# stcodeer/Frequency-wised_All-in-One_Image_Restoration_Model

Measured on AMD Instinct MI355X. Metric: training images/sec @128x128, higher is better.
Workload: dtype bf16; 1 GPU; BASELINE configs[1]: Uformer encoder+decoder (all_3_bands, L=3, freq MSA), denoise sigma=25, 128x128, phase-2 train step (fwd+bwd+Adam, DropPath on); per_gpu_batch=16, global_batch=16, parallelism=dp1, hip_graph=True

## Files before the change

### frequency-wised_all-in-one_image_restoration_model_amd/csrc/fw_common.h

```cpp
#pragma once
#include <hip/hip_runtime.h>
#include <stdint.h>
#include <mutex>

#define FW_DT_F32 0
#define FW_DT_BF16 1

typedef __attribute__((ext_vector_type(4))) float f32x4;
typedef __attribute__((ext_vector_type(8))) __bf16 bf16x8_t;
typedef unsigned short bf16raw;

#define FW_DEV static __device__ __forceinline__
#define FW_SPEC __device__ __forceinline__
#define FW_MEM __device__ __forceinline__

FW_DEV int lane_id() { return threadIdx.x & 63; }

FW_DEV float bf2f(bf16raw b) { return __uint_as_float(((unsigned)b) << 16); }
FW_DEV bf16raw f2bf(float f) {
    __bf16 h = (__bf16)f;
    return __builtin_bit_cast(bf16raw, h);
}
typedef __attribute__((ext_vector_type(2))) float fw_f32x2;
typedef __attribute__((ext_vector_type(2))) __bf16 fw_bf16x2;
FW_DEV unsigned pack_bf2(float lo, float hi) {
    const fw_f32x2 v = {lo, hi};
    return __builtin_bit_cast(unsigned, __builtin_convertvector(v, fw_bf16x2));
}

template <typename T> struct TT;
template <> struct TT<float> {
    static constexpr int SZ = 4;
    static constexpr int E16 = 4;
    FW_DEV float ld(const float* p) { return *p; }
    FW_DEV void st(float* p, float v) { *p = v; }
};
template <> struct TT<bf16raw> {
    static constexpr int SZ = 2;
    static constexpr int E16 = 8;
    FW_DEV float ld(const bf16raw* p) { return bf2f(*p); }
    FW_DEV void st(bf16raw* p, float v) { *p = f2bf(v); }
};

template <typename T> FW_DEV void unpack16(const uint4& v, float* f);
template <> FW_SPEC void unpack16<float>(const uint4& v, float* f) {
    f[0] = __uint_as_float(v.x); f[1] = __uint_as_float(v.y);
    f[2] = __uint_as_float(v.z); f[3] = __uint_as_float(v.w);
}
template <> FW_SPEC void unpack16<bf16raw>(const uint4& v, float* f) {
    f[0] = __uint_as_float(v.x << 16); f[1] = __uint_as_float(v.x & 0xffff0000u);
    f[2] = __uint_as_float(v.y << 16); f[3] = __uint_as_float(v.y & 0xffff0000u);
    f[4] = __uint_as_float(v.z << 16); f[5] = __uint_as_float(v.z & 0xffff0000u);
    f[6] = __uint_as_float(v.w << 16); f[7] = __uint_as_float(v.w & 0xffff0000u);
}
template <typename T> FW_DEV uint4 pack16(const float* f);
template <> FW_SPEC uint4 pack16<float>(const float* f) {
    return make_uint4(__float_as_uint(f[0]), __float_as_uint(f[1]), __float_as_uint(f[2]), __float_as_uint(f[3]));
}
template <> FW_SPEC uint4 pack16<bf16raw>(const float* f) {
    return make_uint4(pack_bf2(f[0], f[1]), pack_bf2(f[2], f[3]), pack_bf2(f[4], f[5]), pack_bf2(f[6], f[7]));
}

FW_DEV float erf_fast(float x) {
    const float ax = fabsf(x);
    const float t = __builtin_amdgcn_rcpf(1.0f + 0.3275911f * ax);
    const float poly = t * (0.254829592f + t * (-0.284496736f + t * (1.421413741f + t * (-1.453152027f + t * 1.061405429f))));
    const float r = 1.0f - poly * __expf(-ax * ax);
    return copysignf(r, x);
}
FW_DEV float gelu_f(float x) { return 0.5f * x * (1.0f + erf_fast(x * 0.70710678118654752440f)); }
FW_DEV float gelu_grad_f(float x) {
    const float cdf = 0.5f * (1.0f + erf_fast(x * 0.70710678118654752440f));
    const float pdf = 0.39894228040143267794f * __expf(-0.5f * x * x);
    return cdf + x * pdf;
}
FW_DEV float gelu_poly(float x) {
    const float xc = __builtin_amdgcn_fmed3f(x, -4.0f, 4.0f);
    const float u = xc * xc;
    float p = -1.301290697e-09f;
    p = fmaf(p, u, 1.041962340e-07f); p = fmaf(p, u, -3.657149647e-06f); p = fmaf(p, u, 7.485542814e-05f);
    p = fmaf(p, u, -1.006494109e-03f); p = fmaf(p, u, 9.505412949e-03f); p = fmaf(p, u, -6.588785358e-02f);
    p = fmaf(p, u, 3.986733717e-01f);
    return x * fmaf(xc, p, 0.5f);
}
FW_DEV float gelu_grad_poly(float x) {
    const float xc = __builtin_amdgcn_fmed3f(x, -4.0f, 4.0f);
    const float u = xc * xc;
    float r = -1.641741003e-08f;
    r = fmaf(r, u, 1.213663647e-06f); r = fmaf(r, u, -3.845618281e-05f); r = fmaf(r, u, 6.876052189e-04f);
    r = fmaf(r, u, -7.687198903e-03f); r = fmaf(r, u, 5.591419208e-02f); r = fmaf(r, u, -2.620297180e-01f);
    r = fmaf(r, u, 7.967230048e-01f);
    return fmaf(xc, r, 0.5f);
}
template <typename T> FW_DEV float gelu_t(float x) { return sizeof(T) == 2 ? gelu_poly(x) : gelu_f(x); }
template <typename T> FW_DEV float gelu_grad_t(float x) { return sizeof(T) == 2 ? gelu_grad_poly(x) : gelu_grad_f(x); }
FW_DEV float lrelu_f(float x, float s) { return x > 0.f ? x : x * s; }

FW_DEV float wave_sum(float v) {
#pragma unroll
    for (int o = 32; o > 0; o >>= 1) v += __shfl_xor(v, o, 64);
    return v;
}
FW_DEV float wave_max(float v) {
#pragma unroll
    for (int o = 32; o > 0; o >>= 1) v = fmaxf(v, __shfl_xor(v, o, 64));
    return v;
}

FW_DEV unsigned fw_hash32(unsigned x) {
    x ^= x >> 16; x *= 0x7feb352dU; x ^= x >> 15; x *= 0x846ca68bU; x ^= x >> 16;
    return x;
}
FW_DEV unsigned fw_site_key(unsigned seed, unsigned site) { return fw_hash32(seed ^ fw_hash32(site * 0x9E3779B9U + 0x7F4A7C15U)); }
FW_DEV bool fw_keep(unsigned key, unsigned long long idx, unsigned thresh) {
    return fw_hash32(fw_hash32((unsigned)idx ^ key) + (unsigned)(idx >> 32)) >= thresh;
}
static inline unsigned fw_drop_thresh(float p) {
    const double t = (double)p * 4294967296.0;
    return t <= 0.0 ? 0u : (t >= 4294967295.0 ? 4294967295u : (unsigned)t);
}

template <typename T> FW_DEV void mma_chunk(f32x4& acc, const uint4& a, const uint4& b);
template <> FW_SPEC void mma_chunk<bf16raw>(f32x4& acc, const uint4& a, const uint4& b) {
    acc = __builtin_amdgcn_mfma_f32_16x16x32_bf16(__builtin_bit_cast(bf16x8_t, a),
                                                  __builtin_bit_cast(bf16x8_t, b), acc, 0, 0, 0);
}
template <> FW_SPEC void mma_chunk<float>(f32x4& acc, const uint4& a, const uint4& b) {
    acc = __builtin_amdgcn_mfma_f32_16x16x4f32(__uint_as_float(a.x), __uint_as_float(b.x), acc, 0, 0, 0);
    acc = __builtin_amdgcn_mfma_f32_16x16x4f32(__uint_as_float(a.y), __uint_as_float(b.y), acc, 0, 0, 0);
    acc = __builtin_amdgcn_mfma_f32_16x16x4f32(__uint_as_float(a.z), __uint_as_float(b.z), acc, 0, 0, 0);
    acc = __builtin_amdgcn_mfma_f32_16x16x4f32(__uint_as_float(a.w), __uint_as_float(b.w), acc, 0, 0, 0);
}

FW_DEV uint4 frag_kc(const char* tile, int ldb, int row0, int chunk) {
    const int l = lane_id();
    return *reinterpret_cast<const uint4*>(tile + (row0 + (l & 15)) * ldb + chunk * 64 + ((l >> 4) << 4));
}

template <typename T> FW_DEV uint4 frag_km(const char* tile, int ldb, int m0, int chunk);
template <> FW_SPEC uint4 frag_km<float>(const char* tile, int ldb, int m0, int chunk) {
    const int l = lane_id();
    const char* p = tile + (chunk * 16 + ((l >> 4) << 2)) * ldb + (m0 + (l & 15)) * 4;
    uint4 r;
    r.x = *reinterpret_cast<const unsigned*>(p);
    r.y = *reinterpret_cast<const unsigned*>(p + ldb);
    r.z = *reinterpret_cast<const unsigned*>(p + 2 * ldb);
    r.w = *reinterpret_cast<const unsigned*>(p + 3 * ldb);
    return r;
}
typedef __attribute__((ext_vector_type(4))) short fw_s16x4;
typedef __attribute__((address_space(3))) fw_s16x4 fw_lds_s16x4;
template <> FW_SPEC uint4 frag_km<bf16raw>(const char* tile, int ldb, int m0, int chunk) {
    const int l = lane_id();
    const char* p = tile + (chunk * 32 + ((l >> 4) << 3) + ((l >> 2) & 3)) * ldb + (m0 + ((l & 3) << 2)) * 2;
    const uint2 lo = __builtin_bit_cast(uint2, __builtin_amdgcn_ds_read_tr16_b64_v4i16((fw_lds_s16x4*)p));
    const uint2 hi = __builtin_bit_cast(uint2, __builtin_amdgcn_ds_read_tr16_b64_v4i16((fw_lds_s16x4*)(p + 4 * ldb)));
    return make_uint4(lo.x, lo.y, hi.x, hi.y);
}

template <typename T> FW_DEV void store_acc_T(char* dst, int ldb, int row0, int col0, const f32x4& acc);
template <> FW_SPEC void store_acc_T<float>(char* dst, int ldb, int row0, int col0, const f32x4& acc) {
    const int l = lane_id();
    *reinterpret_cast<f32x4*>(dst + (col0 + (l & 15)) * ldb + (row0 + ((l >> 4) << 2)) * 4) = acc;
}
template <> FW_SPEC void store_acc_T<bf16raw>(char* dst, int ldb, int row0, int col0, const f32x4& acc) {
    const int l = lane_id();
    uint2 v = make_uint2(pack_bf2(acc[0], acc[1]), pack_bf2(acc[2], acc[3]));
    *reinterpret_cast<uint2*>(dst + (col0 + (l & 15)) * ldb + (row0 + ((l >> 4) << 2)) * 2) = v;
}
template <typename T> FW_DEV void store_acc_N(char* dst, int ldb, int row0, int col0, const f32x4& acc) {
    const int l = lane_id();
    char* p = dst + (row0 + ((l >> 4) << 2)) * ldb + (col0 + (l & 15)) * TT<T>::SZ;
#pragma unroll
    for (int r = 0; r < 4; ++r) TT<T>::st(reinterpret_cast<T*>(p + r * ldb), acc[r]);
}

template <typename T, int MT, int NT>
FW_DEV void mma_tiles(f32x4 (&acc)[MT][NT], const char* A, int lda, int a_row0, const char* B, int ldb,
// ... 41 lines not shown
```

### frequency-wised_all-in-one_image_restoration_model_amd/csrc/fw_elem.hip

```cpp
#include "fw_common.h"
#include <stdlib.h>

namespace {

constexpr int TPB = 256;
FW_DEV long gtid() { return (long)blockIdx.x * TPB + threadIdx.x; }
FW_DEV long gstride() { return (long)gridDim.x * TPB; }
static inline int grid_for(long n, int cap = 8192) { long g = (n + TPB - 1) / TPB; return (int)(g < 1 ? 1 : (g > cap ? cap : g)); }

template <typename T> FW_DEV void ldvec(const T* p, float* f) {
    unpack16<T>(*reinterpret_cast<const uint4*>(p), f);
}
template <typename T> FW_DEV void stvec(T* p, const float* f) { *reinterpret_cast<uint4*>(p) = pack16<T>(f); }
template <typename T> FW_DEV void ldvec4(const T* p, float* f);
template <> FW_SPEC void ldvec4<float>(const float* p, float* f) { unpack16<float>(*reinterpret_cast<const uint4*>(p), f); }
template <> FW_SPEC void ldvec4<bf16raw>(const bf16raw* p, float* f) {
    const uint2 v = *reinterpret_cast<const uint2*>(p);
    f[0] = __uint_as_float(v.x << 16); f[1] = __uint_as_float(v.x & 0xffff0000u);
    f[2] = __uint_as_float(v.y << 16); f[3] = __uint_as_float(v.y & 0xffff0000u);
}
template <typename T> FW_DEV void stvec4(T* p, const float* f);
template <> FW_SPEC void stvec4<float>(float* p, const float* f) { *reinterpret_cast<uint4*>(p) = pack16<float>(f); }
template <> FW_SPEC void stvec4<bf16raw>(bf16raw* p, const float* f) {
    *reinterpret_cast<uint2*>(p) = make_uint2(pack_bf2(f[0], f[1]), pack_bf2(f[2], f[3]));
}

template <typename T>
__global__ void cast_rows_kernel(const float* __restrict__ src, long lds_, T* __restrict__ dst, long ldd, long rows, int cols,
                                 const float* __restrict__ rowscale, int rps) {
    const int c4n = cols >> 2;
    for (long i = gtid(); i < rows * c4n; i += gstride()) {
        const long r = i / c4n; const int c = (int)(i % c4n) * 4;
        const f32x4 v = *reinterpret_cast<const f32x4*>(src + r * lds_ + c);
        const float s = rowscale ? rowscale[r / rps] : 1.f;
        T* d = dst + r * ldd + c;
        if (sizeof(T) == 4) *reinterpret_cast<f32x4*>(d) = v * s;
        else *reinterpret_cast<uint2*>(d) = make_uint2(pack_bf2(v[0] * s, v[1] * s), pack_bf2(v[2] * s, v[3] * s));
    }
}
__global__ void copy_rows_kernel(const float* __restrict__ src, long lds_, float* __restrict__ dst, long ldd, long rows, int cols, int acc) {
    const int c4n = cols >> 2;
    for (long i = gtid(); i < rows * c4n; i += gstride()) {
        const long r = i / c4n; const int c = (int)(i % c4n) * 4;
        f32x4 v = *reinterpret_cast<const f32x4*>(src + r * lds_ + c);
        if (acc) v += *reinterpret_cast<const f32x4*>(dst + r * ldd + c);
        *reinterpret_cast<f32x4*>(dst + r * ldd + c) = v;
    }
}
template <typename T>
__global__ void add_rows_kernel(const T* __restrict__ src, long lds_, T* __restrict__ dst, long ldd, long rows, int cols) {
    const int c4n = cols >> 2;
    for (long i = gtid(); i < rows * c4n; i += gstride()) {
        const long r = i / c4n; const int c = (int)(i % c4n) * 4;
        for (int e = 0; e < 4; ++e) {
            T* d = dst + r * ldd + c + e;
            TT<T>::st(d, TT<T>::ld(d) + TT<T>::ld(src + r * lds_ + c + e));
        }
    }
}
template <typename T>
__global__ void cast_flat_kernel(const float* __restrict__ src, T* __restrict__ dst, long n) {
    for (long i = gtid(); i < n; i += gstride()) TT<T>::st(dst + i, src[i]);
}
template <typename TI, typename TO>
__global__ void permute3_kernel(const TI* __restrict__ in, TO* __restrict__ out, int d0, int d1, int d2, long s0, long s1, long s2, int acc) {
    const long n = (long)d0 * d1 * d2;
    for (long i = gtid(); i < n; i += gstride()) {
        const int c = (int)(i % d2); const long t = i / d2; const int b = (int)(t % d1); const int a = (int)(t / d1);
        const long o = a * s0 + b * s1 + c * s2;
        float v = TT<TI>::ld(in + i);
        if (acc) v += TT<TO>::ld(out + o);
        TT<TO>::st(out + o, v);
    }
}

__global__ __launch_bounds__(256) void permute3_multi_kernel(const long long* __restrict__ tab, const long long* __restrict__ prefix, int num) {
    int lo = 0, hi = num;
    while (hi - lo > 1) {
        const int mid = (lo + hi) >> 1;
        if (prefix[mid] <= (long long)blockIdx.x) lo = mid; else hi = mid;
    }
    const long long* t = tab + (long)lo * 10;
    const float* src = reinterpret_cast<const float*>(t[0]);
    const int d1 = (int)t[3], d2 = (int)t[4];
// ... 240 lines not shown
    float gw[10][E];
#pragma unroll
    for (int k = 0; k < 10; ++k)
#pragma unroll
        for (int e = 0; e < E; ++e) gw[k][e] = 0.f;
    if (live)
        for (long s = s0; s < nstrips && s < s0 + NSTRIP; ++s) {
            const int sx = (int)(s % ns); const int y = (int)((s / ns) % H); const long b = s / ((long)ns * H);
            const int x0 = sx * SX;
            const bool left_ok = x0 > 0, right_ok = x0 + SX < W;
            const int xl = left_ok ? x0 - 1 : 0, xr = right_ok ? x0 + SX : W - 1;
            Raw4<T> rg[SX], raw[3][SX + 2];
            const T* grow = g1 + ((b * H + y) * W + x0) * ld1 + c0;
#pragma unroll
            for (int o = 0; o < SX; ++o) rg[o].load(grow + (long)o * ld1);
#pragma unroll
            for (int ky = 0; ky < 3; ++ky) {
                int yy = y - ky + 1;
                yy = yy < 0 ? 0 : (yy >= H ? H - 1 : yy);
                const T* row = dh2 + ((b * H + yy) * W) * ldg + c0;
                raw[ky][0].load(row + (long)xl * ldg);
#pragma unroll
                for (int cx = 0; cx < SX; ++cx) raw[ky][cx + 1].load(row + (long)(x0 + cx) * ldg);
                raw[ky][SX + 1].load(row + (long)xr * ldg);
            }
            float g[SX][E];
#pragma unroll
            for (int o = 0; o < SX; ++o) {
                rg[o].unpack(g[o]);
                if constexpr (GIN) {
#pragma unroll
                    for (int e = 0; e < E; ++e) g[o][e] = gelu_t<T>(g[o][e]);
                }
            }
#pragma unroll
            for (int ky = 0; ky < 3; ++ky) {
                const bool row_ok = (y - ky + 1 >= 0) && (y - ky + 1 < H);
#pragma unroll
                for (int j = 0; j < SX + 2; ++j) {
                    Raw4<T> r = raw[ky][j];
                    r.zero_unless(row_ok && (j >= 1 || left_ok) && (j <= SX || right_ok));
                    float d[E];
                    r.unpack(d);
                    if (ky == 1 && j >= 1 && j <= SX) {
#pragma unroll
                        for (int e = 0; e < E; ++e) gw[9][e] += d[e];
                    }
#pragma unroll
                    for (int kx = 0; kx < 3; ++kx) {
                        const int i = j + kx - 2;
                        if (i >= 0 && i < SX) {
#pragma unroll
                            for (int e = 0; e < E; ++e) gw[ky * 3 + kx][e] += g[i][e] * d[e];
                        }
                    }
                }
            }
        }
    __syncthreads();
#pragma unroll
    for (int k = 0; k < 10; ++k)
#pragma unroll
        for (int e = 0; e < E; ++e) {
            float sum = gw[k][e];
            sum += __shfl_xor(sum, 32, 64);
            if ((threadIdx.x & 63) < WG_VL) atomicAdd(&red[(vl * E + e) * 10 + k], sum);
        }
    __syncthreads();
    for (int i = threadIdx.x; i < WG_VL * E * 10; i += 256) {
        const int k = i % 10, ce = i / 10;
        const int c = (blockIdx.x % nvg) * WG_VL * E + ce;
        if (c < C) {
            if (k < 9) atomicAdd(dw + (long)c * 9 + k, red[i]);
            else atomicAdd(dbias + c, red[i]);
        }
    }
}

template <typename T, bool GIN>
__global__ __launch_bounds__(256, 3) void dwconv_fwd_pipe_kernel(const T* __restrict__ in, long ldi, const float* __restrict__ w, const float* __restrict__ bias,
                                                              T* __restrict__ out, T* __restrict__ out2, long ldo, int B, int H, int W, int C, int NT) {
    constexpr int SZ = TT<T>::SZ, E16 = TT<T>::E16;
    constexpr int PXB = DT_CB * SZ, ROWB = (DT_TX + 2) * PXB + 128, CHUNKS = PXB / 16;
    constexpr int NPIECE = (DT_TY + 2) * (DT_TX + 2) * CHUNKS, NI = (NPIECE + 255) / 256;
    constexpr int TILEB = (DT_TY + 2) * ROWB;
    extern __shared__ __attribute__((aligned(16))) char dsm[];
    const int ncb = (C + DT_CB - 1) / DT_CB, ntx = (W + DT_TX - 1) / DT_TX, nty = H / DT_TY;
    const int ncol = ncb * ntx;
    const long nrow = (long)B * nty, nchunk = (nrow + NT - 1) / NT;
    long bid = blockIdx.x;
    if ((gridDim.x & 7) == 0) bid = (long)(blockIdx.x & 7) * (gridDim.x >> 3) + (blockIdx.x >> 3);
    const int col = (int)(bid % ncol);
    const long chunk = bid / ncol;
    if (chunk >= nchunk) return;
    const int cb = col % ncb, tx = col / ncb;
    const long s0 = chunk * NT, s1 = s0 + NT < nrow ? s0 + NT : nrow;
    const int x0 = tx * DT_TX, c0b = cb * DT_CB;
    int ppack[NI], pxo[NI];
    unsigned pokm = 0;
#pragma unroll
    for (int i = 0; i < NI; ++i) {
        const int idx = threadIdx.x + i * 256;
        const int ch = idx % CHUNKS, px = (idx / CHUNKS) % (DT_TX + 2), row = (idx / (CHUNKS * (DT_TX + 2))) % (DT_TY + 2);
        int xx = x0 + px - 1, cc = c0b + ch * E16;
        if (idx < NPIECE && xx >= 0 && xx < W && cc + E16 <= C) pokm |= 1u << i;
        xx = xx < 0 ? 0 : (xx >= W ? W - 1 : xx); cc = cc + E16 <= C ? cc : 0;
        pxo[i] = xx * (int)ldi + cc; ppack[i] = (row * ROWB + px * PXB + ch * 16) | (row << 24);
    }
    const int cv = threadIdx.x & 15, ry = (threadIdx.x >> 4) & 7, sxl = threadIdx.x >> 7;
    const int c0 = c0b + cv * 4;
    const bool c_ok = c0 + 4 <= C;
    const int cw = c_ok ? c0 : 0;
    const int ox0 = x0 + sxl * 8;
    float* wl = reinterpret_cast<float*>(dsm + TILEB);
    for (int i = threadIdx.x; i < 9 * DT_CB; i += 256) {
        const int c = c0b + (i % DT_CB);
        wl[i] = c < C ? w[(i / DT_CB) * C + c] : 0.f;
    }
    const f32x4 b4 = *reinterpret_cast<const f32x4*>(bias + cw);
    const int rowelems = W * (int)ldi;
    uint4 r[NI];
    auto issue = [&](long s) {
        const T* base = in + (s / nty) * H * (long)rowelems;
        const int y0 = (int)(s % nty) * DT_TY;
#pragma unroll
        for (int i = 0; i < NI; ++i) {
            int yy = y0 + (ppack[i] >> 24) - 1;
            yy = yy < 0 ? 0 : (yy >= H ? H - 1 : yy);
            r[i] = *reinterpret_cast<const uint4*>(base + (yy * rowelems + pxo[i]));
        }
    };
    issue(s0);
    for (long s = s0; s < s1; ++s) {
        const long b = s / nty;
        const int y0 = (int)(s % nty) * DT_TY;
#pragma unroll
        for (int i = 0; i < NI; ++i) {
            if (threadIdx.x + i * 256 >= NPIECE) continue;
            const int yy = y0 + (ppack[i] >> 24) - 1;
            uint4 piece = r[i];
            if constexpr (GIN) {
                float f[E16];
                unpack16<T>(piece, f);
#pragma unroll
                for (int e = 0; e < E16; ++e) f[e] = gelu_t<T>(f[e]);
                piece = pack16<T>(f);
            }
            *reinterpret_cast<uint4*>(dsm + (ppack[i] & 0xffffff)) = (((pokm >> i) & 1) && yy >= 0 && yy < H) ? piece : make_uint4(0, 0, 0, 0);
            __builtin_amdgcn_sched_barrier(0);
        }
        __syncthreads();
        if (s + 1 < s1) issue(s + 1);
        float acc[8][4];
#pragma unroll
        for (int o = 0; o < 8; ++o)
#pragma unroll
            for (int e = 0; e < 4; ++e) acc[o][e] = b4[e];
#pragma unroll 1
        for (int ky = 0; ky < 3; ++ky) {
            const char* rowp = dsm + (ry + ky) * ROWB + (sxl * 8) * PXB + cv * 4 * SZ;
            f32x4 wk[3];
#pragma unroll
            for (int kx = 0; kx < 3; ++kx) wk[kx] = *reinterpret_cast<const f32x4*>(wl + (ky * 3 + kx) * DT_CB + cv * 4);
#pragma unroll
            for (int cx = 0; cx < 10; ++cx) {
                Raw4<T> q;
                q.lds(rowp + cx * PXB);
                float f[4];
                q.unpack(f);
#pragma unroll
                for (int kx = 0; kx < 3; ++kx) {
                    const int o = cx - kx;
                    if (o >= 0 && o < 8) {
#pragma unroll
                        for (int e = 0; e < 4; ++e) acc[o][e] += f[e] * wk[kx][e];
                    }
                }
            }
        }
        const long tok0 = ((b * H + y0 + ry) * W + ox0) * ldo + c0;
#pragma unroll
        for (int o = 0; o < 8; ++o) {
            const bool ok = c_ok && ox0 + o < W;
            if (ok) stvec4<T>(out + tok0 + (long)o * ldo, acc[o]);
#pragma unroll
            for (int e = 0; e < 4; ++e) acc[o][e] = gelu_t<T>(acc[o][e]);
            if (ok) stvec4<T>(out2 + tok0 + (long)o * ldo, acc[o]);
        }
        __syncthreads();
    }
}

template <typename T>
__global__ __launch_bounds__(256, 2) void dwconv_bwd_fused_kernel(const T* __restrict__ dh2, long ldg, const T* __restrict__ h1, const float* __restrict__ w,
                                                               T* __restrict__ dh1, long ldo, float* __restrict__ dw, float* __restrict__ dbias,
                                                               int B, int H, int W, int C, int NT) {
    constexpr int SZ = TT<T>::SZ, E16 = TT<T>::E16;
    constexpr int PXB = DT_CB * SZ, ROWB = (DT_TX + 2) * PXB + 128, CHUNKS = PXB / 16;
    constexpr int NPIECE = (DT_TY + 2) * (DT_TX + 2) * CHUNKS, NI = (NPIECE + 255) / 256;
    extern __shared__ __attribute__((aligned(16))) char dsm[];
    const int ncb = (C + DT_CB - 1) / DT_CB, ntx = (W + DT_TX - 1) / DT_TX, nty = H / DT_TY;
    const int ncol = ncb * ntx;
    const long nrow = (long)B * nty, nchunk = (nrow + NT - 1) / NT;
    long bid = blockIdx.x;
    if ((gridDim.x & 7) == 0) bid = (long)(blockIdx.x & 7) * (gridDim.x >> 3) + (blockIdx.x >> 3);
    const int col = (int)(bid % ncol);
    const long chunk = bid / ncol;
    if (chunk >= nchunk) return;
    const int cb = col % ncb, tx = col / ncb;
    const long s0 = chunk * NT, s1 = s0 + NT < nrow ? s0 + NT : nrow;
    const int x0 = tx * DT_TX, c0b = cb * DT_CB;
    int ppack[NI], pxo[NI];
    unsigned pokm = 0;
#pragma unroll
    for (int i = 0; i < NI; ++i) {
        const int idx = threadIdx.x + i * 256;
        const int ch = idx % CHUNKS, px = (idx / CHUNKS) % (DT_TX + 2), row = (idx / (CHUNKS * (DT_TX + 2))) % (DT_TY + 2);
        int xx = x0 + px - 1, cc = c0b + ch * E16;
        if (idx < NPIECE && xx >= 0 && xx < W && cc + E16 <= C) pokm |= 1u << i;
        xx = xx < 0 ? 0 : (xx >= W ? W - 1 : xx); cc = cc + E16 <= C ? cc : 0;
        pxo[i] = xx * (int)ldg + cc; ppack[i] = (row * ROWB + px * PXB + ch * 16) | (row << 24);
    }
    const int cv = threadIdx.x & 15, ry = (threadIdx.x >> 4) & 7, sxl = threadIdx.x >> 7;
    const int c0 = c0b + cv * 4;
    const bool c_ok = c0 + 4 <= C;
    const int cw = c_ok ? c0 : 0;
    const int ox0 = x0 + sxl * 8;
    constexpr int TILEB = (DT_TY + 2) * ROWB;
    float* wl = reinterpret_cast<float*>(dsm + TILEB);
    float* part = wl + 9 * DT_CB;
    for (int i = threadIdx.x; i < 9 * DT_CB; i += 256) {
        const int k = i / DT_CB, c = c0b + (i % DT_CB);
        wl[i] = c < C ? w[(8 - k) * C + c] : 0.f;
    }
#pragma unroll
    for (int j = 0; j < 40; ++j) part[j * 256 + threadIdx.x] = 0.f;
    float gb[4] = {0.f, 0.f, 0.f, 0.f};
    uint4 r[NI];
    Raw4<T> pre[8];
    const int rowelems = W * (int)ldg;
    auto issue_halo = [&](long s) {
        const T* base = dh2 + (s / nty) * H * (long)rowelems;
        const int y0 = (int)(s % nty) * DT_TY;
#pragma unroll
        for (int i = 0; i < NI; ++i) {
            int yy = y0 + (ppack[i] >> 24) - 1;
            yy = yy < 0 ? 0 : (yy >= H ? H - 1 : yy);
            r[i] = *reinterpret_cast<const uint4*>(base + (yy * rowelems + pxo[i]));
        }
    };
    auto issue_pre = [&](long s) {
        const T* base = h1 + (s / nty) * H * (long)rowelems;
        const int yoff = ((int)(s % nty) * DT_TY + ry) * rowelems + cw;
#pragma unroll
        for (int o = 0; o < 8; ++o) {
            const int xx = ox0 + o < W ? ox0 + o : W - 1;
            pre[o].load(base + (yoff + xx * (int)ldg));
        }
    };
    issue_halo(s0);
    issue_pre(s0);
    for (long s = s0; s < s1; ++s) {
        const long b = s / nty;
        const int y0 = (int)(s % nty) * DT_TY;
#pragma unroll
        for (int i = 0; i < NI; ++i) {
            if (threadIdx.x + i * 256 >= NPIECE) continue;
            const int yy = y0 + (ppack[i] >> 24) - 1;
            *reinterpret_cast<uint4*>(dsm + (ppack[i] & 0xffffff)) = (((pokm >> i) & 1) && yy >= 0 && yy < H) ? r[i] : make_uint4(0, 0, 0, 0);
        }
        __syncthreads();
        float g[8][4], acc[8][4];
#pragma unroll
        for (int o = 0; o < 8; ++o) {
            float hc[4];
            pre[o].unpack(hc);
            const bool in = ox0 + o < W;
#pragma unroll
            for (int e = 0; e < 4; ++e) { g[o][e] = in ? gelu_t<T>(hc[e]) : 0.f; acc[o][e] = 0.f; }
            if (o & 1) __builtin_amdgcn_sched_barrier(0);
        }
#pragma unroll 1
        for (int ky = 0; ky < 3; ++ky) {
            const char* rowp = dsm + (ry + ky) * ROWB + (sxl * 8) * PXB + cv * 4 * SZ;
            f32x4 wk[3];
            float gk[3][4];
#pragma unroll
            for (int kx = 0; kx < 3; ++kx) {
                wk[kx] = *reinterpret_cast<const f32x4*>(wl + (ky * 3 + kx) * DT_CB + cv * 4);
#pragma unroll
                for (int e = 0; e < 4; ++e) gk[kx][e] = 0.f;
            }
            const float bsel = ky == 1 ? 1.f : 0.f;
#pragma unroll
            for (int cx = 0; cx < 10; ++cx) {
                Raw4<T> q;
                q.lds(rowp + cx * PXB);
                float f[4];
                q.unpack(f);
                if (cx >= 1 && cx <= 8) {
#pragma unroll
                    for (int e = 0; e < 4; ++e) gb[e] += bsel * f[e];
                }
#pragma unroll
                for (int kx = 0; kx < 3; ++kx) {
                    const int o = cx - kx;
                    if (o >= 0 && o < 8) {
#pragma unroll
                        for (int e = 0; e < 4; ++e) {
                            acc[o][e] += f[e] * wk[kx][e];
                            gk[kx][e] += f[e] * g[o][e];
                        }
                    }
                }
                if (cx == 4) __builtin_amdgcn_sched_barrier(0);
            }
#pragma unroll
            for (int kx = 0; kx < 3; ++kx)
#pragma unroll
                for (int e = 0; e < 4; ++e) part[((ky * 3 + kx) * 4 + e) * 256 + threadIdx.x] += gk[kx][e];
        }
        __builtin_amdgcn_sched_barrier(0);
        if (s + 1 < s1) issue_halo(s + 1);
        __builtin_amdgcn_sched_barrier(0);
        T* orow = dh1 + ((b * H + y0 + ry) * W + ox0) * ldo + c0;
#pragma unroll
        for (int o = 0; o < 8; ++o) {
            float hc[4];
            Raw4<T> again = pre[o];
            again.launder();
            again.unpack(hc);
#pragma unroll
            for (int e = 0; e < 4; ++e) acc[o][e] *= gelu_grad_t<T>(hc[e]);
            if (c_ok && ox0 + o < W) stvec4<T>(orow + (long)o * ldo, acc[o]);
            if (o & 1) __builtin_amdgcn_sched_barrier(0);
        }
        if (s + 1 < s1) issue_pre(s + 1);
        __syncthreads();
    }
    float* red = reinterpret_cast<float*>(dsm);
    const int wave = threadIdx.x >> 6;
#pragma unroll
    for (int j = 0; j < 40; ++j) {
        float v = j < 36 ? part[j * 256 + threadIdx.x] : gb[j - 36];
        v += __shfl_xor(v, 16, 64);
        v += __shfl_xor(v, 32, 64);
        if ((threadIdx.x & 63) < 16) red[(wave * 16 + cv) * 40 + j] = v;
    }
    __syncthreads();
    for (int i = threadIdx.x; i < 16 * 40; i += 256) {
        const int cvv = i / 40, j = i % 40, k = j >> 2, e = j & 3;
        const float sum = red[cvv * 40 + j] + red[(16 + cvv) * 40 + j] + red[(32 + cvv) * 40 + j] + red[(48 + cvv) * 40 + j];
        const int c = c0b + cvv * 4 + e;
        if (c < C) {
            if (k < 9) atomicAdd(dw + (long)c * 9 + (8 - k), sum);
            else atomicAdd(dbias + c, sum);
        }
    }
}

template <typename T>
__global__ void im2col4_kernel(const float* __restrict__ x, long ldx, T* __restrict__ col, int B, int H, int W, int C) {
    const int Ho = H / 2, Wo = W / 2, c4n = C >> 2;
    const long total = (long)B * Ho * Wo * 16 * c4n;
    for (long i = gtid(); i < total; i += gstride()) {
        const int c = (int)(i % c4n) * 4; long t = i / c4n;
        const int tap = (int)(t % 16); t /= 16;
        const int ox = (int)(t % Wo); const int oy = (int)((t / Wo) % Ho); const long b = t / ((long)Wo * Ho);
        const int iy = 2 * oy - 1 + (tap >> 2), ix = 2 * ox - 1 + (tap & 3);
        f32x4 v = f32x4{0.f, 0.f, 0.f, 0.f};
        if (iy >= 0 && iy < H && ix >= 0 && ix < W) v = *reinterpret_cast<const f32x4*>(x + ((b * H + iy) * W + ix) * ldx + c);
        T* d = col + (t * 16 + tap) * (long)C + c;
        if (sizeof(T) == 4) *reinterpret_cast<f32x4*>(d) = v;
        else *reinterpret_cast<uint2*>(d) = make_uint2(pack_bf2(v[0], v[1]), pack_bf2(v[2], v[3]));
    }
}
template <typename T>
__global__ void col2im4_kernel(const T* __restrict__ dcol, float* __restrict__ dx, long lddx, const float* __restrict__ dres, long ldr,
                               int B, int H, int W, int C) {
    const int Ho = H / 2, Wo = W / 2, c4n = C >> 2;
    const long total = (long)B * H * W * c4n;
    for (long i = gtid(); i < total; i += gstride()) {
        const int c = (int)(i % c4n) * 4; const long tok = i / c4n;
        const int x = (int)(tok % W); const int y = (int)((tok / W) % H); const long b = tok / ((long)W * H);
        f32x4 acc = f32x4{0.f, 0.f, 0.f, 0.f};
        if (dres) acc = *reinterpret_cast<const f32x4*>(dres + tok * ldr + c);
        for (int ky = (y + 1) & 1; ky < 4; ky += 2) {
            const int oy = (y + 1 - ky) / 2;
            if (y + 1 - ky < 0 || oy >= Ho) continue;
            for (int kx = (x + 1) & 1; kx < 4; kx += 2) {
                const int ox = (x + 1 - kx) / 2;
                if (x + 1 - kx < 0 || ox >= Wo) continue;
                const T* s = dcol + (((b * Ho + oy) * Wo + ox) * 16 + ky * 4 + kx) * (long)C + c;
                for (int e = 0; e < 4; ++e) acc[e] += TT<T>::ld(s + e);
            }
        }
        *reinterpret_cast<f32x4*>(dx + tok * lddx + c) = acc;
    }
}

template <typename T>
__global__ void pixel_shuffle_kernel(const T* __restrict__ g, const float* __restrict__ bias, float* __restrict__ out, long ldo,
                                     int B, int H, int W, int Cout) {
    const int c4n = Cout >> 2;
    const long total = (long)B * H * W * 4 * c4n;
    for (long i = gtid(); i < total; i += gstride()) {
        const int c = (int)(i % c4n) * 4; long t = i / c4n;
        const int q = (int)(t % 4); t /= 4;
        const int x = (int)(t % W); const int y = (int)((t / W) % H); const long b = t / ((long)W * H);
        const T* s = g + t * 4L * Cout + q * Cout + c;
        float* d = out + ((b * 2 * H + 2 * y + (q >> 1)) * 2 * W + 2 * x + (q & 1)) * ldo + c;
        f32x4 v;
        for (int e = 0; e < 4; ++e) v[e] = TT<T>::ld(s + e) + bias[c + e];
        *reinterpret_cast<f32x4*>(d) = v;
    }
}
template <typename T>
// ... 744 lines not shown
```

Baseline: 329.2 images/sec.

## Reuse halo rows via LDS ring buffer and packed fp32x2 math in dwconv kernels

The depthwise conv forward and backward pipeline kernels now keep the tile rows in an LDS ring buffer. When walking down the image they load only the DT_TY new rows and reuse the two overlap rows from the previous tile, loading a full top halo only at the first tile or at an image start. The stencil FMAs, the GELU polynomials and the GELU-gradient polynomials are rewritten on 2-wide float vectors so the compiler can emit packed fp32 instructions. The bias-grad row accumulation is specialised per ky so the bsel multiply is dropped for bf16. This cuts redundant global loads and ALU instruction count, but adds ring-index arithmetic and more complex control flow.

```diff
diff --git a/frequency-wised_all-in-one_image_restoration_model_amd/csrc/fw_common.h b/frequency-wised_all-in-one_image_restoration_model_amd/csrc/fw_common.h
--- a/frequency-wised_all-in-one_image_restoration_model_amd/csrc/fw_common.h
+++ b/frequency-wised_all-in-one_image_restoration_model_amd/csrc/fw_common.h
@@ -94,6 +94,53 @@
 }
 template <typename T> FW_DEV float gelu_t(float x) { return sizeof(T) == 2 ? gelu_poly(x) : gelu_f(x); }
 template <typename T> FW_DEV float gelu_grad_t(float x) { return sizeof(T) == 2 ? gelu_grad_poly(x) : gelu_grad_f(x); }
+FW_DEV fw_f32x2 fw_fma2(fw_f32x2 a, fw_f32x2 b, fw_f32x2 c) { return __builtin_elementwise_fma(a, b, c); }
+FW_DEV fw_f32x2 gelu_poly2(fw_f32x2 x) {
+    const fw_f32x2 xc = {__builtin_amdgcn_fmed3f(x[0], -4.0f, 4.0f), __builtin_amdgcn_fmed3f(x[1], -4.0f, 4.0f)};
+    const fw_f32x2 u = xc * xc;
+#define FW_S2(c) (fw_f32x2{c, c})
+    fw_f32x2 p = FW_S2(-1.301290697e-09f);
+    p = fw_fma2(p, u, FW_S2(1.041962340e-07f)); p = fw_fma2(p, u, FW_S2(-3.657149647e-06f)); p = fw_fma2(p, u, FW_S2(7.485542814e-05f));
+    p = fw_fma2(p, u, FW_S2(-1.006494109e-03f)); p = fw_fma2(p, u, FW_S2(9.505412949e-03f)); p = fw_fma2(p, u, FW_S2(-6.588785358e-02f));
+    p = fw_fma2(p, u, FW_S2(3.986733717e-01f));
+    return x * fw_fma2(xc, p, FW_S2(0.5f));
+#undef FW_S2
+}
+FW_DEV fw_f32x2 gelu_grad_poly2(fw_f32x2 x) {
+    const fw_f32x2 xc = {__builtin_amdgcn_fmed3f(x[0], -4.0f, 4.0f), __builtin_amdgcn_fmed3f(x[1], -4.0f, 4.0f)};
+    const fw_f32x2 u = xc * xc;
+#define FW_S2(c) (fw_f32x2{c, c})
+    fw_f32x2 r = FW_S2(-1.641741003e-08f);
+    r = fw_fma2(r, u, FW_S2(1.213663647e-06f)); r = fw_fma2(r, u, FW_S2(-3.845618281e-05f)); r = fw_fma2(r, u, FW_S2(6.876052189e-04f));
+    r = fw_fma2(r, u, FW_S2(-7.687198903e-03f)); r = fw_fma2(r, u, FW_S2(5.591419208e-02f)); r = fw_fma2(r, u, FW_S2(-2.620297180e-01f));
+    r = fw_fma2(r, u, FW_S2(7.967230048e-01f));
+    return fw_fma2(xc, r, FW_S2(0.5f));
+#undef FW_S2
+}
+template <typename T, int N> FW_DEV void gelu_grad_vec(float* f) {
+    if constexpr (sizeof(T) == 2) {
+#pragma unroll
+        for (int e = 0; e < N; e += 2) {
+            const fw_f32x2 v = gelu_grad_poly2(fw_f32x2{f[e], f[e + 1]});
+            f[e] = v[0]; f[e + 1] = v[1];
+        }
+    } else {
+#pragma unroll
+        for (int e = 0; e < N; ++e) f[e] = gelu_grad_f(f[e]);
+    }
+}
+template <typename T, int N> FW_DEV void gelu_vec(float* f) {
+    if constexpr (sizeof(T) == 2) {
+#pragma unroll
+        for (int e = 0; e < N; e += 2) {
+            const fw_f32x2 v = gelu_poly2(fw_f32x2{f[e], f[e + 1]});
+            f[e] = v[0]; f[e + 1] = v[1];
+        }
+    } else {
+#pragma unroll
+        for (int e = 0; e < N; ++e) f[e] = gelu_f(f[e]);
+    }
+}
 FW_DEV float lrelu_f(float x, float s) { return x > 0.f ? x : x * s; }
 
 FW_DEV float wave_sum(float v) {
diff --git a/frequency-wised_all-in-one_image_restoration_model_amd/csrc/fw_elem.hip b/frequency-wised_all-in-one_image_restoration_model_amd/csrc/fw_elem.hip
--- a/frequency-wised_all-in-one_image_restoration_model_amd/csrc/fw_elem.hip
+++ b/frequency-wised_all-in-one_image_restoration_model_amd/csrc/fw_elem.hip
@@ -1,5 +1,6 @@
 #include "fw_common.h"
 #include <stdlib.h>
+#include <type_traits>
 
 namespace {
 
@@ -406,8 +407,10 @@
                                                               T* __restrict__ out, T* __restrict__ out2, long ldo, int B, int H, int W, int C, int NT) {
     constexpr int SZ = TT<T>::SZ, E16 = TT<T>::E16;
     constexpr int PXB = DT_CB * SZ, ROWB = (DT_TX + 2) * PXB + 128, CHUNKS = PXB / 16;
-    constexpr int NPIECE = (DT_TY + 2) * (DT_TX + 2) * CHUNKS, NI = (NPIECE + 255) / 256;
-    constexpr int TILEB = (DT_TY + 2) * ROWB;
+    constexpr int RPIECE = (DT_TX + 2) * CHUNKS, NRING = DT_TY + 2;
+    constexpr int NNEW = DT_TY * RPIECE, NI = (NNEW + 255) / 256;
+    constexpr int NTOP = 2 * RPIECE, NJ = (NTOP + 255) / 256;
+    constexpr int TILEB = NRING * ROWB;
     extern __shared__ __attribute__((aligned(16))) char dsm[];
     const int ncb = (C + DT_CB - 1) / DT_CB, ntx = (W + DT_TX - 1) / DT_TX, nty = H / DT_TY;
     const int ncol = ncb * ntx;
@@ -425,11 +428,11 @@
 #pragma unroll
     for (int i = 0; i < NI; ++i) {
         const int idx = threadIdx.x + i * 256;
-        const int ch = idx % CHUNKS, px = (idx / CHUNKS) % (DT_TX + 2), row = (idx / (CHUNKS * (DT_TX + 2))) % (DT_TY + 2);
+        const int ch = idx % CHUNKS, px = (idx / CHUNKS) % (DT_TX + 2), row = 2 + (idx / RPIECE) % DT_TY;
         int xx = x0 + px - 1, cc = c0b + ch * E16;
-        if (idx < NPIECE && xx >= 0 && xx < W && cc + E16 <= C) pokm |= 1u << i;
+        if (idx < NNEW && xx >= 0 && xx < W && cc + E16 <= C) pokm |= 1u << i;
         xx = xx < 0 ? 0 : (xx >= W ? W - 1 : xx); cc = cc + E16 <= C ? cc : 0;
-        pxo[i] = xx * (int)ldi + cc; ppack[i] = (row * ROWB + px * PXB + ch * 16) | (row << 24);
+        pxo[i] = xx * (int)ldi + cc; ppack[i] = (px * PXB + ch * 16) | (row << 24);
     }
     const int cv = threadIdx.x & 15, ry = (threadIdx.x >> 4) & 7, sxl = threadIdx.x >> 7;
     const int c0 = c0b + cv * 4;
@@ -450,54 +453,86 @@
 #pragma unroll
         for (int i = 0; i < NI; ++i) {
             int yy = y0 + (ppack[i] >> 24) - 1;
-            yy = yy < 0 ? 0 : (yy >= H ? H - 1 : yy);
+            yy = yy >= H ? H - 1 : yy;
             r[i] = *reinterpret_cast<const uint4*>(base + (yy * rowelems + pxo[i]));
+        }
+    };
+    auto put = [&](uint4 piece, bool ok, int off) {
+        if constexpr (GIN) {
+            float f[E16];
+            unpack16<T>(piece, f);
+            gelu_vec<T, E16>(f);
+            piece = pack16<T>(f);
+        }
+        *reinterpret_cast<uint4*>(dsm + off) = ok ? piece : make_uint4(0, 0, 0, 0);
+    };
+    auto stage_top = [&](long s) {
+        const T* base = in + (s / nty) * H * (long)rowelems;
+        const int y0 = (int)(s % nty) * DT_TY;
+        uint4 q[NJ];
+#pragma unroll
+        for (int j = 0; j < NJ; ++j) {
+            const int idx = threadIdx.x + j * 256;
+            const int ch = idx % CHUNKS, px = (idx / CHUNKS) % (DT_TX + 2), row = (idx / RPIECE) & 1;
+            int xx = x0 + px - 1, cc = c0b + ch * E16, yy = y0 + row - 1;
+            xx = xx < 0 ? 0 : (xx >= W ? W - 1 : xx); cc = cc + E16 <= C ? cc : 0; yy = yy < 0 ? 0 : yy;
+            q[j] = *reinterpret_cast<const uint4*>(base + (yy * rowelems + xx * (int)ldi + cc));
+        }
+#pragma unroll
+        for (int j = 0; j < NJ; ++j) {
+            const int idx = threadIdx.x + j * 256;
+            if (idx >= NTOP) continue;
+            const int ch = idx % CHUNKS, px = (idx / CHUNKS) % (DT_TX + 2), row = idx / RPIECE;
+            const int xx = x0 + px - 1, cc = c0b + ch * E16;
+            put(q[j], xx >= 0 && xx < W && cc + E16 <= C && y0 + row - 1 >= 0, row * ROWB + px * PXB + ch * 16);
         }
     };
     issue(s0);
+    int rbase = 0;
     for (long s = s0; s < s1; ++s) {
         const long b = s / nty;
-        const int y0 = (int)(s % nty) * DT_TY;
+        const int ty = (int)(s % nty), y0 = ty * DT_TY;
+        const bool full = s == s0 || ty == 0;
+        rbase = full ? 0 : (rbase >= 2 ? rbase - 2 : rbase + DT_TY);
 #pragma unroll
         for (int i = 0; i < NI; ++i) {
-            if (threadIdx.x + i * 256 >= NPIECE) continue;
-            const int yy = y0 + (ppack[i] >> 24) - 1;
-            uint4 piece = r[i];
-            if constexpr (GIN) {
-                float f[E16];
-                unpack16<T>(piece, f);
-#pragma unroll
-                for (int e = 0; e < E16; ++e) f[e] = gelu_t<T>(f[e]);
-                piece = pack16<T>(f);
-            }
-            *reinterpret_cast<uint4*>(dsm + (ppack[i] & 0xffffff)) = (((pokm >> i) & 1) && yy >= 0 && yy < H) ? piece : make_uint4(0, 0, 0, 0);
+            if (threadIdx.x + i * 256 >= NNEW) continue;
+            const int row = ppack[i] >> 24;
+            int slot = rbase + row;
+            slot = slot >= NRING ? slot - NRING : slot;
+            put(r[i], ((pokm >> i) & 1) && y0 + row - 1 < H, slot * ROWB + (ppack[i] & 0xffffff));
             __builtin_amdgcn_sched_barrier(0);
         }
+        if (full) stage_top(s);
         __syncthreads();
         if (s + 1 < s1) issue(s + 1);
-        float acc[8][4];
-#pragma unroll
-        for (int o = 0; o < 8; ++o)
-#pragma unroll
-            for (int e = 0; e < 4; ++e) acc[o][e] = b4[e];
+        fw_f32x2 acc[8][2];
+#pragma unroll
+        for (int o = 0; o < 8; ++o) { acc[o][0] = fw_f32x2{b4[0], b4[1]}; acc[o][1] = fw_f32x2{b4[2], b4[3]}; }
 #pragma unroll 1
         for (int ky = 0; ky < 3; ++ky) {
-            const char* rowp = dsm + (ry + ky) * ROWB + (sxl * 8) * PXB + cv * 4 * SZ;
-            f32x4 wk[3];
-#pragma unroll
-            for (int kx = 0; kx < 3; ++kx) wk[kx] = *reinterpret_cast<const f32x4*>(wl + (ky * 3 + kx) * DT_CB + cv * 4);
+            int slot = rbase + ry + ky;
+            slot = slot >= NRING ? slot - NRING : slot;
+            const char* rowp = dsm + slot * ROWB + (sxl * 8) * PXB + cv * 4 * SZ;
+            fw_f32x2 wk[3][2];
+#pragma unroll
+            for (int kx = 0; kx < 3; ++kx) {
+                const f32x4 w4 = *reinterpret_cast<const f32x4*>(wl + (ky * 3 + kx) * DT_CB + cv * 4);
+                wk[kx][0] = fw_f32x2{w4[0], w4[1]}; wk[kx][1] = fw_f32x2{w4[2], w4[3]};
+            }
 #pragma unroll
             for (int cx = 0; cx < 10; ++cx) {
                 Raw4<T> q;
                 q.lds(rowp + cx * PXB);
                 float f[4];
                 q.unpack(f);
+                const fw_f32x2 f2[2] = {fw_f32x2{f[0], f[1]}, fw_f32x2{f[2], f[3]}};
 #pragma unroll
                 for (int kx = 0; kx < 3; ++kx) {
                     const int o = cx - kx;
                     if (o >= 0 && o < 8) {
-#pragma unroll
-                        for (int e = 0; e < 4; ++e) acc[o][e] += f[e] * wk[kx][e];
+                        acc[o][0] = fw_fma2(f2[0], wk[kx][0], acc[o][0]);
+                        acc[o][1] = fw_fma2(f2[1], wk[kx][1], acc[o][1]);
                     }
                 }
             }
@@ -506,10 +541,10 @@
 #pragma unroll
         for (int o = 0; o < 8; ++o) {
             const bool ok = c_ok && ox0 + o < W;
-            if (ok) stvec4<T>(out + tok0 + (long)o * ldo, acc[o]);
-#pragma unroll
-            for (int e = 0; e < 4; ++e) acc[o][e] = gelu_t<T>(acc[o][e]);
-            if (ok) stvec4<T>(out2 + tok0 + (long)o * ldo, acc[o]);
+            float a[4] = {acc[o][0][0], acc[o][0][1], acc[o][1][0], acc[o][1][1]};
+            if (ok) stvec4<T>(out + tok0 + (long)o * ldo, a);
+            gelu_vec<T, 4>(a);
+            if (ok) stvec4<T>(out2 + tok0 + (long)o * ldo, a);
         }
         __syncthreads();
     }
@@ -521,7 +556,9 @@
                                                                int B, int H, int W, int C, int NT) {
     constexpr int SZ = TT<T>::SZ, E16 = TT<T>::E16;
     constexpr int PXB = DT_CB * SZ, ROWB = (DT_TX + 2) * PXB + 128, CHUNKS = PXB / 16;
-    constexpr int NPIECE = (DT_TY + 2) * (DT_TX + 2) * CHUNKS, NI = (NPIECE + 255) / 256;
+    constexpr int RPIECE = (DT_TX + 2) * CHUNKS, NRING = DT_TY + 2;
+    constexpr int NNEW = DT_TY * RPIECE, NI = (NNEW + 255) / 256;
+    constexpr int NTOP = 2 * RPIECE, NJ = (NTOP + 255) / 256;
     extern __shared__ __attribute__((aligned(16))) char dsm[];
     const int ncb = (C + DT_CB - 1) / DT_CB, ntx = (W + DT_TX - 1) / DT_TX, nty = H / DT_TY;
     const int ncol = ncb * ntx;
@@ -539,18 +576,18 @@
 #pragma unroll
     for (int i = 0; i < NI; ++i) {
         const int idx = threadIdx.x + i * 256;
-        const int ch = idx % CHUNKS, px = (idx / CHUNKS) % (DT_TX + 2), row = (idx / (CHUNKS * (DT_TX + 2))) % (DT_TY + 2);
+        const int ch = idx % CHUNKS, px = (idx / CHUNKS) % (DT_TX + 2), row = 2 + (idx / RPIECE) % DT_TY;
         int xx = x0 + px - 1, cc = c0b + ch * E16;
-        if (idx < NPIECE && xx >= 0 && xx < W && cc + E16 <= C) pokm |= 1u << i;
+        if (idx < NNEW && xx >= 0 && xx < W && cc + E16 <= C) pokm |= 1u << i;
         xx = xx < 0 ? 0 : (xx >= W ? W - 1 : xx); cc = cc + E16 <= C ? cc : 0;
-        pxo[i] = xx * (int)ldg + cc; ppack[i] = (row * ROWB + px * PXB + ch * 16) | (row << 24);
+        pxo[i] = xx * (int)ldg + cc; ppack[i] = (px * PXB + ch * 16) | (row << 24);
     }
     const int cv = threadIdx.x & 15, ry = (threadIdx.x >> 4) & 7, sxl = threadIdx.x >> 7;
     const int c0 = c0b + cv * 4;
     const bool c_ok = c0 + 4 <= C;
     const int cw = c_ok ? c0 : 0;
     const int ox0 = x0 + sxl * 8;
-    constexpr int TILEB = (DT_TY + 2) * ROWB;
+    constexpr int TILEB = NRING * ROWB;
     float* wl = reinterpret_cast<float*>(dsm + TILEB);
     float* part = wl + 9 * DT_CB;
     for (int i = threadIdx.x; i < 9 * DT_CB; i += 256) {
@@ -558,7 +595,7 @@
         wl[i] = c < C ? w[(8 - k) * C + c] : 0.f;
     }
 #pragma unroll
-    for (int j = 0; j < 40; ++j) part[j * 256 + threadIdx.x] = 0.f;
+    for (int j = 0; j < 36; ++j) part[j * 256 + threadIdx.x] = 0.f;
     float gb[4] = {0.f, 0.f, 0.f, 0.f};
     uint4 r[NI];
     Raw4<T> pre[8];
@@ -569,8 +606,30 @@
 #pragma unroll
         for (int i = 0; i < NI; ++i) {
             int yy = y0 + (ppack[i] >> 24) - 1;
-            yy = yy < 0 ? 0 : (yy >= H ? H - 1 : yy);
+            yy = yy >= H ? H - 1 : yy;
             r[i] = *reinterpret_cast<const uint4*>(base + (yy * rowelems + pxo[i]));
+        }
+    };
+    auto stage_top = [&](long s) {
+        const T* base = dh2 + (s / nty) * H * (long)rowelems;
+        const int y0 = (int)(s % nty) * DT_TY;
+        uint4 q[NJ];
+#pragma unroll
+        for (int j = 0; j < NJ; ++j) {
+            const int idx = threadIdx.x + j * 256;
+            const int ch = idx % CHUNKS, px = (idx / CHUNKS) % (DT_TX + 2), row = (idx / RPIECE) & 1;
+            int xx = x0 + px - 1, cc = c0b + ch * E16, yy = y0 + row - 1;
+            xx = xx < 0 ? 0 : (xx >= W ? W - 1 : xx); cc = cc + E16 <= C ? cc : 0; yy = yy < 0 ? 0 : yy;
+            q[j] = *reinterpret_cast<const uint4*>(base + (yy * rowelems + xx * (int)ldg + cc));
+        }
+#pragma unroll
+        for (int j = 0; j < NJ; ++j) {
+            const int idx = threadIdx.x + j * 256;
+            if (idx >= NTOP) continue;
+            const int ch = idx % CHUNKS, px = (idx / CHUNKS) % (DT_TX + 2), row = idx / RPIECE;
+            const int xx = x0 + px - 1, cc = c0b + ch * E16;
+            *reinterpret_cast<uint4*>(dsm + row * ROWB + px * PXB + ch * 16) =
+                (xx >= 0 && xx < W && cc + E16 <= C && y0 + row - 1 >= 0) ? q[j] : make_uint4(0, 0, 0, 0);
         }
     };
     auto issue_pre = [&](long s) {
@@ -584,56 +643,69 @@
     };
     issue_halo(s0);
     issue_pre(s0);
+    int rbase = 0;
     for (long s = s0; s < s1; ++s) {
         const long b = s / nty;
-        const int y0 = (int)(s % nty) * DT_TY;
+        const int ty = (int)(s % nty), y0 = ty * DT_TY;
+        const bool full = s == s0 || ty == 0;
+        rbase = full ? 0 : (rbase >= 2 ? rbase - 2 : rbase + DT_TY);
 #pragma unroll
         for (int i = 0; i < NI; ++i) {
-            if (threadIdx.x + i * 256 >= NPIECE) continue;
-            const int yy = y0 + (ppack[i] >> 24) - 1;
-            *reinterpret_cast<uint4*>(dsm + (ppack[i] & 0xffffff)) = (((pokm >> i) & 1) && yy >= 0 && yy < H) ? r[i] : make_uint4(0, 0, 0, 0);
-        }
+            if (threadIdx.x + i * 256 >= NNEW) continue;
+            const int row = ppack[i] >> 24;
+            int slot = rbase + row;
+            slot = slot >= NRING ? slot - NRING : slot;
+            *reinterpret_cast<uint4*>(dsm + slot * ROWB + (ppack[i] & 0xffffff)) = (((pokm >> i) & 1) && y0 + row - 1 < H) ? r[i] : make_uint4(0, 0, 0, 0);
+        }
+        if (full) stage_top(s);
         __syncthreads();
-        float g[8][4], acc[8][4];
+        fw_f32x2 g[8][2], acc[8][2];
 #pragma unroll
         for (int o = 0; o < 8; ++o) {
             float hc[4];
             pre[o].unpack(hc);
+            gelu_vec<T, 4>(hc);
             const bool in = ox0 + o < W;
 #pragma unroll
-            for (int e = 0; e < 4; ++e) { g[o][e] = in ? gelu_t<T>(hc[e]) : 0.f; acc[o][e] = 0.f; }
+            for (int h = 0; h < 2; ++h) {
+                g[o][h] = in ? fw_f32x2{hc[2 * h], hc[2 * h + 1]} : fw_f32x2{0.f, 0.f};
+                acc[o][h] = fw_f32x2{0.f, 0.f};
+            }
             if (o & 1) __builtin_amdgcn_sched_barrier(0);
         }
-#pragma unroll 1
-        for (int ky = 0; ky < 3; ++ky) {
-            const char* rowp = dsm + (ry + ky) * ROWB + (sxl * 8) * PXB + cv * 4 * SZ;
-            f32x4 wk[3];
-            float gk[3][4];
+        fw_f32x2 gb2[2] = {fw_f32x2{gb[0], gb[1]}, fw_f32x2{gb[2], gb[3]}};
+        auto stencil_row = [&](int ky, auto mode) {
+            int slot = rbase + ry + ky;
+            slot = slot >= NRING ? slot - NRING : slot;
+            const char* rowp = dsm + slot * ROWB + (sxl * 8) * PXB + cv * 4 * SZ;
+            fw_f32x2 wk[3][2], gk[3][2];
 #pragma unroll
             for (int kx = 0; kx < 3; ++kx) {
-                wk[kx] = *reinterpret_cast<const f32x4*>(wl + (ky * 3 + kx) * DT_CB + cv * 4);
-#pragma unroll
-                for (int e = 0; e < 4; ++e) gk[kx][e] = 0.f;
+                const f32x4 w4 = *reinterpret_cast<const f32x4*>(wl + (ky * 3 + kx) * DT_CB + cv * 4);
+                wk[kx][0] = fw_f32x2{w4[0], w4[1]}; wk[kx][1] = fw_f32x2{w4[2], w4[3]};
+                gk[kx][0] = gk[kx][1] = fw_f32x2{0.f, 0.f};
             }
-            const float bsel = ky == 1 ? 1.f : 0.f;
 #pragma unroll
             for (int cx = 0; cx < 10; ++cx) {
                 Raw4<T> q;
                 q.lds(rowp + cx * PXB);
                 float f[4];
                 q.unpack(f);
-                if (cx >= 1 && cx <= 8) {
-#pragma unroll
-                    for (int e = 0; e < 4; ++e) gb[e] += bsel * f[e];
+                const fw_f32x2 f2[2] = {fw_f32x2{f[0], f[1]}, fw_f32x2{f[2], f[3]}};
+                if constexpr (decltype(mode)::value == 1) {
+                    if (cx >= 1 && cx <= 8) { gb2[0] += f2[0]; gb2[1] += f2[1]; }
+                } else if constexpr (decltype(mode)::value == 2) {
+                    const float bsel = ky == 1 ? 1.f : 0.f;
+                    if (cx >= 1 && cx <= 8) { gb2[0] = fw_fma2(fw_f32x2{bsel, bsel}, f2[0], gb2[0]); gb2[1] = fw_fma2(fw_f32x2{bsel, bsel}, f2[1], gb2[1]); }
                 }
 #pragma unroll
                 for (int kx = 0; kx < 3; ++kx) {
                     const int o = cx - kx;
                     if (o >= 0 && o < 8) {
 #pragma unroll
-                        for (int e = 0; e < 4; ++e) {
-                            acc[o][e] += f[e] * wk[kx][e];
-                            gk[kx][e] += f[e] * g[o][e];
+                        for (int h = 0; h < 2; ++h) {
+                            acc[o][h] = fw_fma2(f2[h], wk[kx][h], acc[o][h]);
+                            gk[kx][h] = fw_fma2(f2[h], g[o][h], gk[kx][h]);
                         }
                     }
                 }
@@ -642,8 +714,16 @@
 #pragma unroll
             for (int kx = 0; kx < 3; ++kx)
 #pragma unroll
-                for (int e = 0; e < 4; ++e) part[((ky * 3 + kx) * 4 + e) * 256 + threadIdx.x] += gk[kx][e];
-        }
+                for (int e = 0; e < 4; ++e) part[((ky * 3 + kx) * 4 + e) * 256 + threadIdx.x] += gk[kx][e >> 1][e & 1];
+        };
+#pragma unroll 1
+        for (int ky = 0; ky < 3; ++ky) {
+            if constexpr (sizeof(T) == 2) {
+                if (ky == 1) stencil_row(ky, std::integral_constant<int, 1>{});
+                else stencil_row(ky, std::integral_constant<int, 0>{});
+            } else stencil_row(ky, std::integral_constant<int, 2>{});
+        }
+        gb[0] = gb2[0][0]; gb[1] = gb2[0][1]; gb[2] = gb2[1][0]; gb[3] = gb2[1][1];
         __builtin_amdgcn_sched_barrier(0);
         if (s + 1 < s1) issue_halo(s + 1);
         __builtin_amdgcn_sched_barrier(0);
@@ -654,9 +734,10 @@
             Raw4<T> again = pre[o];
             again.launder();
             again.unpack(hc);
-#pragma unroll
-            for (int e = 0; e < 4; ++e) acc[o][e] *= gelu_grad_t<T>(hc[e]);
-            if (c_ok && ox0 + o < W) stvec4<T>(orow + (long)o * ldo, acc[o]);
+            gelu_grad_vec<T, 4>(hc);
+            const fw_f32x2 d0 = acc[o][0] * fw_f32x2{hc[0], hc[1]}, d1 = acc[o][1] * fw_f32x2{hc[2], hc[3]};
+            const float a[4] = {d0[0], d0[1], d1[0], d1[1]};
+            if (c_ok && ox0 + o < W) stvec4<T>(orow + (long)o * ldo, a);
             if (o & 1) __builtin_amdgcn_sched_barrier(0);
         }
         if (s + 1 < s1) issue_pre(s + 1);
```

New measurement: 330.3 images/sec (median of 6 runs). No clear change (+0.3%).
